# Monash-Connected-Autonomous-Vehicle/unsupervised-pseuso-LiDAR

Hardware: AMD Instinct MI355X
Metric: images/sec (fwd+bwd) KITTI 192x640 triplets, full training step (higher is better)
Workload: dtype f32; 1 GPU; BASELINE.json configs[1]: per-GPU batch=12, 192x640 KITTI-shaped triplets, ResNet-18 depth encoder + 6-DoF PoseNet, fp32 (the ResNet trunk's 3x3 stride-1 convolutions and their data gradients: fp32 contractions on split operands -- three bf16 planes per operand, six bf16-MFMA plane products, fp32 accumulation; every other launch: fp32 MFMA), one step = 2x depth fwd + pose fwd + warp/L1/smooth loss; global_batch=12, parallelism=dp1

## Files before the change

### unsupervised-pseuso-lidar_amd/csrc/conv_bf16.hip

```cpp
#include "conv_shared.h"
#include "kernel_timer.h"

namespace mcav {

typedef __bf16 bf16x8 __attribute__((ext_vector_type(8)));
typedef __bf16 bf16x4 __attribute__((ext_vector_type(4)));
typedef __bf16 bf16x2 __attribute__((ext_vector_type(2)));
typedef unsigned short u16;
typedef unsigned int u32x2 __attribute__((ext_vector_type(2)));

template <int BM_, int BN_, int WM_, int WN_, int MF_, int CK_>
struct BTile {
    static constexpr int BM = BM_, BN = BN_, WM = WM_, WN = WN_, MF = MF_;
    static constexpr int KD = CK_;
    static constexpr int LDH = CK_ + 8;
    static constexpr int LPRA = CK_ / 4;
    static constexpr int RPPA = 256 / LPRA;
    static constexpr int AROWS = BM / RPPA;
    static constexpr int LPRB = CK_ / 8;
    static constexpr int BVECS = (BN * LPRB + 255) / 256;
    static constexpr int WAVES_M = BM / WM, WAVES_N = BN / WN;
    static constexpr int TM = WM / MF, TN = WN / MF;
    static constexpr int ACC = MF == 32 ? 16 : 4;
    using AccT = typename std::conditional<MF_ == 32, f32x16, f32x4>::type;
// ... 750 lines not shown
            const bf16x8 zero = {0, 0, 0, 0, 0, 0, 0, 0};
#pragma unroll
            for (int q = 0; q < NS; ++q) {
                const bf16x8 v = *reinterpret_cast<const bf16x8*>(ap + q * APL);
                a[q] = keep ? v : zero;
            }
        };
        const bool yrow = (ky == 0 && has_y1) || (ky == 2 && has_yl);
        const unsigned ybit = ky == 0 ? 1u : 2u;
        const int sky = 2 - ky;
        for (int ks = 0; ks < 2; ++ks) {
            bf16x8 b[3][NS];
#pragma unroll
            for (int kx = 0; kx < 3; ++kx)
#pragma unroll
                for (int q = 0; q < NS; ++q) b[kx][q] = *reinterpret_cast<const bf16x8*>(Bst + (ks ? b_lane1 : b_lane0) + (kx * NS + q) * BPL);
            const unsigned m = rmask;
            bf16x8 a[NS];
            if (has_x1) { afr(ky, 2, ks, a, (m & 4u) != 0); mma(a, b[0]); }
            if (has_xl) { afr(ky, 0, ks, a, (m & 8u) != 0); mma(a, b[2]); }
            if (yrow) {
                const bool my = (m & ybit) != 0;
#pragma unroll
                for (int kx = 0; kx < 3; ++kx) { afr(sky, kx, ks, a, my); mma(a, b[kx]); }
                if (has_x1) { afr(sky, 2, ks, a, my && (m & 4u)); mma(a, b[0]); }
                if (has_xl) { afr(sky, 0, ks, a, my && (m & 8u)); mma(a, b[2]); }
            }
        }
    };
    auto compute = [&](int ky, const u16* Bst) {
        const int rsh = (fwd ? ky : 2 - ky) * PW + (fwd ? 0 : 2);
        const int dxr = fwd ? 1 : -1;
        bf16x8 fa[2][NS], fb[2][NS];
        auto load = [&](int i, bf16x8 (&a)[NS], bf16x8 (&b)[NS]) {
            const int kx = i >> 1, ks = i & 1;
            const u16* const bp = Bst + (ks ? b_lane1 : b_lane0) + kx * NS * BPL;
#pragma unroll
            for (int q = 0; q < NS; ++q) b[q] = *reinterpret_cast<const bf16x8*>(bp + q * BPL);
            const int row = prow + rsh + kx * dxr;
            const u16* const ap = Asub + row * LDH + (((2 * ks + fslot) ^ ((row >> 2) & 3)) * 8);
#pragma unroll
            for (int q = 0; q < NS; ++q) a[q] = *reinterpret_cast<const bf16x8*>(ap + q * APL);
        };
        load(0, fa[0], fb[0]);
#pragma unroll
        for (int i = 0; i < 6; ++i) {
            if (i + 1 < 6) load(i + 1, fa[(i + 1) & 1], fb[(i + 1) & 1]);
            __builtin_amdgcn_sched_barrier(0);
            if (!(diag & 8)) mma(fa[i & 1], fb[i & 1]);
            __builtin_amdgcn_sched_barrier(0);
        }
    };

    f32x4 ra[NJ], rbn[NS];
    const int total = nchunks * 3;
    issueA(ra, 0);
    issueB(rbn, 0);
    storeA(ra);
    storeB(rbn, 0);
    if (total > 1) issueB(rbn, 1);
    __syncthreads();
    int ky = 0, chunk = 0;
    for (int s = 0; s < total; ++s) {
        const bool more = chunk + 1 < nchunks;
        const u16* const Bst = Bs + (s & 1) * BSTAGE;
        if (ky == 0 && more && !(diag & 4)) issueA(ra, chunk + 1);
        compute(ky, Bst);
        if constexpr (ADJ) {
            if (has_y1 | has_yl | has_x1 | has_xl) extras(ky, Bst);
        }
        if (s + 1 < total && !(diag & 1)) {
            storeB(rbn, (s + 1) & 1);
            if (s + 2 < total) issueB(rbn, s + 2);
        }
        if (ky == 2 && more && !(diag & 4)) {
            __syncthreads();
            storeA(ra);
        }
        __syncthreads();
        if (++ky == 3) { ky = 0; ++chunk; }
    }
    if constexpr (NS > 1) acc[0][0] += mid + low;
    if (diag & 16) return;
    igemm_epilogue_lean<T>(p, acc, s_out, s_stat, tid, wm0, wn0, n0, mt);
}

#ifndef MCAV_PATCH2_DIAG
#define MCAV_PATCH2_DIAG 0
#endif

template <int SB, int BN_>
struct Patch2Cfg {
    static constexpr int BM = 64 * SB, BN = BN_;
    static constexpr int PIX = 110;
    static constexpr int VP = SB * PIX;
    static constexpr int NJ = (VP + 31) / 32;
    using T = typename std::conditional<SB == 4, BTile<256, BN_, 64, BN_, 32, 32>, BTile<128, BN_, 32, BN_, 32, 32>>::type;
};

template <int NS, int SB, int BN>
constexpr size_t patch2_lds_bytes() { return sizeof(u16) * (size_t)NS * (SB * 110 + 2 * 3 * BN) * 32 + sizeof(unsigned) * 64 * SB; }

template <int NS, int SB, int BN>
__global__ __launch_bounds__(256, BN == 32 ? 2 : 1) void conv3x3_patch2_kernel(IgemmParams p, const u16* __restrict__ w16, PatchGeo geo) {
    using C = Patch2Cfg<SB, BN>;
    using T = typename C::T;
    constexpr int BM = C::BM, CKT = 32, LDH = 32, PIX = C::PIX, TM = T::TM, TN = T::TN;
    constexpr int APL = PIX * LDH;
    constexpr int BPL = BN * LDH;
    constexpr int BSTAGE = 3 * NS * BPL;
    extern __shared__ __attribute__((aligned(16))) unsigned char s_raw[];
    u16* const Ap = reinterpret_cast<u16*>(s_raw);
    u16* const Bs = Ap + SB * NS * APL;
    unsigned* const s_out = reinterpret_cast<unsigned*>(Bs + 2 * BSTAGE);
    float (*const s_stat)[2][BN] = reinterpret_cast<float (*)[2][BN]>(Bs);
    static_assert(sizeof(u16) * BSTAGE >= sizeof(float) * T::WAVES_M * 2 * BN, "statistics scratch fits a filter stage");

    const int tid = threadIdx.x, lane = tid & 63, wave = tid >> 6;
    const int lid = xcd_remap(blockIdx.x, gridDim.x);
    const int nt = lid % p.ntiles, mt = lid / p.ntiles;
    const int n0 = nt * BN;
    const GatherSrc& g = p.g;
    const int TH = geo.TH, TW = geo.TW, PW = TW + 2, PH = TH + 2;
    const int per_img = geo.tiles_y * geo.tiles_x, nblk = g.B * per_img;

    __shared__ int s_pp[C::PIX];
    if (tid < PIX) {
        const int ppy = tid / PW;
        s_pp[tid] = tid < PH * PW ? (ppy << 8) | (tid - ppy * PW) : -1;
    }
    int sb_base[SB], sb_y0[SB], sb_x0[SB];
#pragma unroll
    for (int sb = 0; sb < SB; ++sb) {
        const int blk = mt * SB + sb;
        const int img = blk / per_img, tr = blk - img * per_img, tyi = tr / geo.tiles_x;
        sb_base[sb] = blk < nblk ? img : -1;
        sb_y0[sb] = tyi * TH;
        sb_x0[sb] = (tr - tyi * geo.tiles_x) * TW;
    }
    {
        const int sbw = tid >> 6;
        if (sbw < SB) {
            unsigned o = OOB;
            int img = -1, y0 = 0, x0 = 0;
#pragma unroll
            for (int sb = 0; sb < SB; ++sb)
                if (sb == sbw) { img = sb_base[sb]; y0 = sb_y0[sb]; x0 = sb_x0[sb]; }
            if (img >= 0) {
                const int pix = patch_pixel(tid & 63);
                const int py = pix / TW, px = pix - py * TW;
                const int y = y0 + py, x = x0 + px;
                if (py < TH && y < p.Hd && x < p.Wd) o = (unsigned)((img * p.Hd + y) * p.Wd + x) * (unsigned)(p.Cd * 4);
            }
            s_out[tid] = o;
        }
    }
    __syncthreads();
    const int c4 = tid & 7, pp0 = tid >> 3;
    unsigned aoff[C::NJ];
#pragma unroll
    for (int j = 0; j < C::NJ; ++j) {
        const int vp = pp0 + 32 * j;
        const int sbj = vp / PIX, pp = vp - sbj * PIX;
        unsigned off = OOB;
        if (vp < C::VP) {
            int img = -1, y0 = 0, x0 = 0;
#pragma unroll
// ... 935 lines not shown
```

### unsupervised-pseuso-lidar_amd/csrc/conv_plan.h

```cpp
#pragma once
#include <stddef.h>
#include <stdlib.h>

#include "../../include/mcav_conv.h"

#ifndef MCAV_OK
#define MCAV_OK 0
#define MCAV_E_INVALID (-1)
#endif
#ifndef MCAV_KNOB_INT
#ifdef MCAV_TUNE_ENV
#define MCAV_KNOB_INT(name, dflt) ([] { const char* e = getenv(name); return e ? atoi(e) : (dflt); }())
#else
#define MCAV_KNOB_INT(name, dflt) (dflt)
#endif
#endif

namespace mcav {

constexpr int CK = 16;
constexpr int KP = 32;
constexpr int KPB = 64;
constexpr int TAB_TAPS = 32;
constexpr int WG_TABCAP = 2048;
constexpr int HT_H = 8, HT_W = 32;
constexpr int ST_TW = 32;
constexpr int ST_TH_DEPTH = 8, ST_TH_POSE = 4;
constexpr int SW_TH = 4;
constexpr int patch_pix(int tmb) { return tmb == 1 ? 110 : 180; }
constexpr int P3_SUBS = 3, P3_PIX = 110;
constexpr int WGP_PIX = 110;
static_assert(P3_PIX == patch_pix(1) && WGP_PIX == patch_pix(1), "the 64-pixel block shape of patch_plan serves every 64-pixel form");

inline int round_up(int v, int a) { return (v + a - 1) / a * a; }
inline int kstride_of(int taps, int Kp) { return round_up(taps * Kp, CK); }

constexpr void tile_dims(int id, int& BM, int& BN) {
    switch (id) {
        case 1: BM = 128; BN = 64; break;
        case 2: BM = 64; BN = 64; break;
        case 3: BM = 256; BN = 32; break;
        case 4: BM = 256; BN = 16; break;
        case 5: BM = 128; BN = 128; break;
        case 7: BM = 128; BN = 32; break;
        case 8: BM = 128; BN = 64; break;
        case 9: BM = 128; BN = 128; break;
        case 10: BM = 64; BN = 64; break;
        case 11: BM = 64; BN = 64; break;
        case 12: BM = 32; BN = 64; break;
        default: BM = 64; BN = 16; break;
    }
}
constexpr int tile_bm(int id) { int BM = 0, BN = 0; tile_dims(id, BM, BN); return BM; }
constexpr int tile_bn(int id) { int BM = 0, BN = 0; tile_dims(id, BM, BN); return BN; }
constexpr int tile_kd(int id) { return (id >= 8 && id <= 10) || id == 12 ? 32 : (id == 11 ? 64 : 16); }
constexpr int tile_arows(int id) { return tile_bm(id) * tile_kd(id) / 1024; }

struct GatherSrc {
    const float* x1;
    const float* x2;
    int B, Hs, Ws, C1, C2, up1;
    int mode, stride, sign, offset, pad_mode;
};

struct IgemmParams {
    GatherSrc g;
    const float* w;
    int kh, kw, Kp, Kstride, taps;
    float* y;
    int Hd, Wd, Cd, n_begin, n_count, y_choff;
    const float* bias;
    int act;
    const float* dact_aux;
    int dact;
    const float* addend;
    int pool;
    float* stats;
    const float *stats_x, *stats_mean, *stats_invstd;
    int M;
    int Mc, McP;
    int groups;
    int mtiles, ntiles;
    int no_tab;
    const float* wm;
    int Np_all;
    int bm;
    int upm;
    int ksplit;
    float* kslab;
};

struct PatchGeo {
    int TH, TW, tiles_y, tiles_x;
    int tmb;
    int refl;
};

struct WgradParams {
    GatherSrc g;
    int kh, kw, Kp, taps, Ktot;
    const float* dy;
    int Hd, Wd, Cdy, dy_choff, Cout;
    int CoutLoad;
    int Mpix;
    int splits, pix_per_split;
    int mtiles, ntiles;
    float* slab;
    int slabN;
    int want_bias;
    int tab_cht_log2;
    int upm;
    int Hf, Wf;
    int split_planes;
    int patch, pTH, pTW, ptiles_y, ptiles_x, prefl, pnblocks, pbps, pct_co, pnarrow;
};

struct WgradPlan {
    WgradParams p;
    int tile;
    bool use_tab;
    bool use_halo;
    bool use_stem;
    size_t slab_bytes, pre_bytes;
    int ci_t, groups, per_group;
};

struct PlanEnv {
    int cus;
};

struct IgemmRoute {
    int family;
    int variant;
    int tile;
    int mtiles, ntiles;
    int workgroups;
    int ksplit;
    PatchGeo geo;
    const mcav_igemm_desc* d;
    mcav_igemm_desc planar_d;
    IgemmParams p;
};

struct WgradRoute {
    int family;
    int variant;
    const mcav_wgrad_desc* d;
    mcav_wgrad_desc planar_d;
    WgradPlan pl;
    int workgroups;
    size_t workspace_bytes() const { return pl.slab_bytes + pl.pre_bytes; }
};

inline int pick_tile(const mcav_igemm_desc* d, long M) {
    if (d->tile) return d->tile;
    if (d->n_count <= 16) return (M >= 256 * 64 && d->kh * d->kw <= 16) ? 4 : 6;
    if (d->n_count <= 32) return 7;
    if (d->mode == MCAV_G_ADJ_REFLECT && ((M + 127) / 128) * ((d->n_count + 63) / 64) >= 1024) return 2;
    if (d->mode != MCAV_G_SMALLC && ((M + 127) / 128) * ((d->n_count + 63) / 64) >= 1024) return 1;
    const long t64 = ((M + 63) / 64) * ((d->n_count + 63) / 64);
    if (d->mode != MCAV_G_SMALLC && d->Kp % 32 == 0 && (t64 <= 128 || (t64 > 256 && t64 < 512))) return 12;
    if (d->mode != MCAV_G_SMALLC && d->Kp % 32 == 0) return 10;
    const long t128x64 = ((M + 127) / 128) * ((d->n_count + 63) / 64);
    return t128x64 >= 1024 ? 1 : 2;
}

inline bool bytes_fit_31(long a, long b, long c, long e) {
    const long lim = 0x7fffffffL;
    if (a <= 0 || b <= 0 || c <= 0 || e <= 0) return false;
    if (a >= lim / b) return false;
    a *= b;
    if (a >= lim / c) return false;
    a *= c;
    return a < lim / e;
}

inline bool prod_below(long lim, long a, long b, long c = 1, long e = 1) { return (unsigned __int128)a * b * c * e < (unsigned __int128)lim; }

inline bool fill_params(const mcav_igemm_desc* d, IgemmParams& p, int& tile) {
    if (!d || !d->x1 || !d->w || !d->y) return false;
    if (d->B <= 0 || d->Hs <= 0 || d->Ws <= 0 || d->Hd <= 0 || d->Wd <= 0 || d->C1 <= 0 || d->C2 < 0) return false;
    if (d->C2 > 0 && !d->x2) return false;
    if (d->kh <= 0 || d->kw <= 0 || d->Np <= 0 || d->Kp <= 0 || d->kh > 64 || d->kw > 64 || d->kh * d->kw > 64) return false;
    if (d->n_begin < 0 || d->n_count <= 0 || d->n_begin > d->Np - d->n_count) return false;
    if (d->Cd <= 0 || d->y_choff < 0 || d->y_choff > d->Cd - d->n_count) return false;
    if (d->mode == MCAV_G_SMALLC) { if (d->Kp != 4 || d->C1 != 4 || d->C2 != 0) return false; }
    else if (d->Kp % CK != 0 || (long)d->Kp < (long)d->C1 + d->C2) return false;
    if (d->C2 > 0 && (d->C1 % 4 != 0)) return false;
    if (d->mode == MCAV_G_ADJ_REFLECT && (d->kh != 3 || d->kw != 3 || d->Hs != d->Hd || d->Ws != d->Wd || d->Hs < 2 || d->Ws < 2)) return false;
    if (d->pad_mode == MCAV_PAD_REFLECT && (d->Hs < 2 || d->Ws < 2)) return false;
    if (d->up1 && ((d->Hs & 1) || (d->Ws & 1))) return false;
    if (d->pool && ((d->Hd & 1) || (d->Wd & 1) || d->mode == MCAV_G_ADJ_STRIDE2)) return false;
    if (d->pool && d->stats) return false;
    if (d->stats_x && (!d->stats || !d->stats_mean || !d->stats_invstd || d->pool || d->y_choff != 0 || d->n_begin != 0 || d->n_count != d->Cd)) return false;
    if (!prod_below(0x7fffffffL, d->B, d->Hs, d->Ws, (long)(d->C1 > d->C2 ? d->C1 : d->C2) * 4)) return false;
    const long kstride = ((long)d->kh * d->kw * d->Kp + CK - 1) / CK * CK;
    if (!prod_below(0x7fffffffL, d->Np, kstride, 4)) return false;
    if (!bytes_fit_31((long)d->B, d->pool ? d->Hd >> 1 : d->Hd, d->pool ? d->Wd >> 1 : d->Wd, (long)d->Cd * 4)) return false;
    p.g.x1 = d->x1; p.g.x2 = d->x2; p.g.B = d->B; p.g.Hs = d->Hs; p.g.Ws = d->Ws; p.g.C1 = d->C1; p.g.C2 = d->C2; p.g.up1 = d->up1;
    p.g.mode = d->mode; p.g.stride = d->stride; p.g.sign = d->sign; p.g.offset = d->offset; p.g.pad_mode = d->pad_mode;
    p.w = d->w; p.kh = d->kh; p.kw = d->kw; p.Kp = d->Kp; p.taps = d->kh * d->kw; p.Kstride = kstride_of(p.taps, d->Kp);
    p.y = d->y; p.Hd = d->Hd; p.Wd = d->Wd; p.Cd = d->Cd; p.n_begin = d->n_begin; p.n_count = d->n_count; p.y_choff = d->y_choff;
    p.bias = d->bias; p.act = d->act; p.dact_aux = d->dact_aux; p.dact = d->dact; p.addend = d->addend; p.pool = d->pool; p.stats = d->stats;
    p.stats_x = d->stats ? d->stats_x : nullptr; p.stats_mean = d->stats_mean; p.stats_invstd = d->stats_invstd;
    const long Mlin = (long)d->B * d->Hd * d->Wd;
    p.no_tab = (d->tile >> 8) & 1;
    p.ksplit = 1; p.kslab = nullptr;
    p.wm = d->w_upmerge; p.Np_all = d->Np; p.upm = 0; p.bm = 0;
    tile = pick_tile(d, Mlin) & 0xff;
    if (tile == 0) { mcav_igemm_desc dd = *d; dd.tile = 0; tile = pick_tile(&dd, Mlin); }
    if (((tile >= 8 && tile <= 10) || tile == 12) && (d->mode == MCAV_G_SMALLC || d->Kp % 32 != 0)) return false;
    if (tile == 11 && (d->mode == MCAV_G_SMALLC || d->Kp % 64 != 0)) return false;
    int BM, BN;
    tile_dims(tile, BM, BN);
    p.groups = d->groups > 1 ? d->groups : 1;
    if (p.groups > 1) {
        if ((d->mode != MCAV_G_DIRECT && d->mode != MCAV_G_SMALLC) || d->pool || d->B % p.groups != 0) return false;
        p.Mc = (int)(Mlin / p.groups);
        p.McP = round_up(p.Mc, BM);
        p.M = p.groups * p.McP;
    } else if (d->mode == MCAV_G_ADJ_STRIDE2) {
        p.Mc = d->B * ((d->Hd + 1) / 2) * ((d->Wd + 1) / 2);
        p.McP = round_up(p.Mc, BM);
        p.M = 4 * p.McP;
    } else {
        p.Mc = 0; p.McP = 1;
        if (Mlin > 0x7fffffffL) return false;
        p.M = (int)Mlin;
        const int ck = tile_kd(tile);
        if (d->w_upmerge && d->mode == MCAV_G_DIRECT && d->kh == 3 && d->kw == 3 && d->stride == 1 && d->sign == 1 && d->offset == -1 &&
            d->pad_mode == MCAV_PAD_REFLECT && d->up1 == 1 && d->C2 > 0 && !(d->Hd & 1) && !(d->Wd & 1) && d->Hd == d->Hs && d->Wd == d->Ws &&
            !d->pool && !d->stats && d->C1 % ck == 0 && d->C2 % ck == 0 && d->C1 + d->C2 == d->Kp && (d->C1 & 3) == 0 && !p.no_tab &&
            (long)4 * d->Np * 4 * d->C1 * 4 < 0x7fffffffL) {
            p.upm = 1;
            p.bm = BM;
            p.Mc = d->B * (d->Hd / 2) * (d->Wd / 2);
            p.McP = round_up(p.Mc, BM);
            p.M = 4 * p.McP;
        }
    }
    p.mtiles = (p.M + BM - 1) / BM;
    p.ntiles = (d->n_count + BN - 1) / BN;
    return true;
}

inline void plan_fp32(IgemmRoute& r) {
    const IgemmParams& p = r.p;
    const int KD = tile_kd(r.tile), AROWS = tile_arows(r.tile);
    const bool c4ok = (p.g.C1 & 3) == 0 && (p.g.C2 & 3) == 0 && (p.g.C2 == 0 || (p.g.C1 & 15) == 0);
    const bool fast_mode = p.g.mode == MCAV_G_DIRECT || (p.g.mode == MCAV_G_ADJ_STRIDE2 && p.g.C2 == 0) || p.g.mode == MCAV_G_SMALLC;
    const bool tab = (p.g.mode == MCAV_G_DIRECT || (p.g.mode == MCAV_G_ADJ_STRIDE2 && p.g.C2 == 0)) && c4ok && p.taps <= TAB_TAPS &&
                     p.g.C1 + p.g.C2 == p.Kp && p.Kp % KD == 0 && (p.g.C2 == 0 || p.g.C1 % KD == 0) && !p.no_tab;
    const bool tab_refl = p.g.mode == MCAV_G_ADJ_REFLECT && c4ok && p.g.C2 == 0 && p.g.C1 == p.Kp && p.Kp % KD == 0 && !p.no_tab && AROWS <= 2;
    r.family = MCAV_IGEMM_FP32;
    r.ksplit = 1;
    if (p.upm) r.variant = MCAV_RV_TABLE | MCAV_RV_UPM;
    else if (tab) r.variant = MCAV_RV_TABLE;
    else if (tab_refl) r.variant = MCAV_RV_TABLE | MCAV_RV_REFLECT | MCAV_RV_ADJ;
    else if (fast_mode && c4ok) r.variant = MCAV_RV_FAST;
    else if (p.g.mode == MCAV_G_ADJ_REFLECT && c4ok && p.g.C2 == 0) r.variant = MCAV_RV_REFLECT | MCAV_RV_ADJ;
    else r.variant = 0;
    if (tab && !p.upm) {
        const bool plain = !p.pool && !p.stats && p.groups <= 1 && p.y_choff == 0 && p.n_count == p.Cd && p.n_begin == 0;
        const int tiles = p.mtiles * p.ntiles, ktiles = p.Kp / KD * p.taps;
        static const int enabled = MCAV_KNOB_INT("MCAV_KSPLIT", 1);
        static const int max_tiles = MCAV_KNOB_INT("MCAV_KSPLIT_TILES", 256);
        if (enabled && plain && tiles <= max_tiles && ktiles >= 32) {
            int ksp = 1024 / tiles;
            if (ksp > 8) ksp = 8;
            if (ksp > ktiles / 4) ksp = ktiles / 4;
            if (ksp >= 2) r.ksplit = ksp;
        }
    }
    r.mtiles = p.mtiles; r.ntiles = p.ntiles;
    r.workgroups = p.mtiles * p.ntiles * r.ksplit;
}

inline bool plan_halo(const mcav_igemm_desc* d, IgemmRoute& r) {
    if (d->kh != 3 || d->kw != 3 || d->stride != 1) return false;
    if (d->C2 != 0 || d->x2 || (d->C1 != 16 && d->C1 != 32) || d->Kp != d->C1) return false;
    if (d->n_count > 32 || d->stats || d->groups > 1 || d->y_choff != 0) return false;
    if (d->Hd != d->Hs || d->Wd != d->Ws || d->Hs < 2 || d->Ws < 2) return false;
    if ((d->tile >> 9) & 1) return false;
    const bool adj = d->mode == MCAV_G_ADJ_REFLECT;
    if (adj) {
        if (d->dact & ~0xff) return false;
        if (d->up1 || d->bias || d->act != MCAV_ACT_NONE) return false;
        if (d->pool && ((d->Hs & 1) || (d->Ws & 1))) return false;
    } else {
        if (d->mode != MCAV_G_DIRECT || d->sign != 1 || d->offset != -1) return false;
// ... 39 lines not shown
        for (int i = 0; i < ns; ++i)
            if (!d->x_planar[i]) return -1;
        return 1;
    }
    if (kind == 2) return d->planar_stack == 2 && d->planar_B == d->B && d->x_planar[1] && d->x_planar[2] ? 1 : -1;
    return -1;
}

inline bool plan_stem(const mcav_igemm_desc* d, bool planar, IgemmRoute& r) {
    const int kind = stem_kind(d);
    if (!kind) return false;
    const int th = kind == 1 ? ST_TH_DEPTH : ST_TH_POSE;
    r.family = MCAV_IGEMM_STEM;
    r.mtiles = d->B * ((d->Hd + th - 1) / th) * ((d->Wd + ST_TW - 1) / ST_TW);
    r.ntiles = 1;
    static const int split_on = MCAV_KNOB_INT("MCAV_STEM_SPLIT", 0);
    const bool split = kind == 1 && (d->mma == 3 || (d->mma == 2 && split_on));
    const bool lean = ((d->tile >> 16) & 1) || kind == 2;
    r.variant = (kind == 2 ? MCAV_RV_POSE : 0) | (planar ? MCAV_RV_PLANAR : 0) | (split ? MCAV_RV_SPLIT : 0) | (lean ? MCAV_RV_LEAN : 0);
    r.workgroups = r.mtiles < (split ? 256 : 512) ? r.mtiles : (split ? 256 : 512);
    return true;
}

inline double patch_block(int H, int W, int rows, int pix, int& TH, int& TW) {
    double best = 1e30;
    TH = 4; TW = 16;
    for (int th = 1; th <= 16; ++th)
        for (int tw = 4; tw <= 64; ++tw) {
            if (th * tw > rows || (th + 2) * (tw + 2) > pix) continue;
            const double tiles = (double)((H + th - 1) / th) * ((W + tw - 1) / tw);
            const double bank = tw % 16 == 0 ? 1.0 : (tw > 16 && tw % 4 == 0 ? 1.05 : 1.25);
            const double cost = tiles * rows * (1.0 + 0.05 * (double)((th + 2) * (tw + 2)) / (th * tw)) * bank;
            if (cost < best) { best = cost; TH = th; TW = tw; }
        }
    return best;
}

struct PatchPlan {
    PatchGeo geo;
    int th1, tw1;
};

inline bool patch_plan(const mcav_igemm_desc* d, PatchPlan& pp, bool f32 = false) {
    PatchGeo& geo = pp.geo;
    static const int enabled = MCAV_KNOB_INT("MCAV_PATCH", 1);
    if (!enabled || !d) return false;
    if (f32 ? (d->mma != 0 || !d->w) : (!d->w16 || d->mma < 1 || d->mma > 3)) return false;
    if (d->kh != 3 || d->kw != 3 || d->stride != 1) return false;
    geo.refl = 0;
    if (d->mode == MCAV_G_DIRECT && d->pad_mode == MCAV_PAD_REFLECT && d->sign == 1 && d->offset == -1) geo.refl = 1;
    else if (d->mode == MCAV_G_ADJ_REFLECT && d->sign == -1 && d->offset == 1) geo.refl = 2;
    else if (d->mode != MCAV_G_DIRECT || d->pad_mode != MCAV_PAD_ZERO) return false;
    else if (!((d->sign == 1 && d->offset == -1) || (d->sign == -1 && d->offset == 1))) return false;
    static const int refl_on = MCAV_KNOB_INT("MCAV_PATCH_REFLECT", 1);
    if (geo.refl && (f32 || d->mma < 2 || !refl_on || d->Hs < 2 || d->Ws < 2)) return false;
    static const int refl_minpix = MCAV_KNOB_INT("MCAV_PATCH_REFLECT_MINPIX", 1000);
    if (geo.refl && d->mma != 3 && (d->n_count < 64 || (geo.refl == 2 && d->Hd * d->Wd < refl_minpix))) return false;
    if (d->C2 != 0 || d->up1 || d->pool || d->w_upmerge) return false;
    if (d->C1 % 32 != 0 || d->Kp != d->C1 || d->Hd != d->Hs || d->Wd != d->Ws || d->n_count < 32) return false;
    if (d->groups > 1 && d->B % d->groups != 0) return false;
    static const int force_tmb = MCAV_KNOB_INT("MCAV_PATCH_TMB", 0);
    int th2, tw2;
    const double c1 = patch_block(d->Hd, d->Wd, 64, patch_pix(1), pp.th1, pp.tw1);
    const double c2 = patch_block(d->Hd, d->Wd, 128, patch_pix(2), th2, tw2);
    const long wg2 = (long)d->B * ((d->Hd + th2 - 1) / th2) * ((d->Wd + tw2 - 1) / tw2) * ((d->n_count + 63) / 64);
    geo.tmb = (c2 <= c1 * 1.02 && wg2 >= 1024) ? 2 : 1;
    if (force_tmb == 1 || force_tmb == 2) geo.tmb = force_tmb;
    geo.TH = geo.tmb == 2 ? th2 : pp.th1;
    geo.TW = geo.tmb == 2 ? tw2 : pp.tw1;
    geo.tiles_y = (d->Hd + geo.TH - 1) / geo.TH;
    geo.tiles_x = (d->Wd + geo.TW - 1) / geo.TW;
    if (d->mma == 1 && (long)d->B * geo.tiles_y * geo.tiles_x * ((d->n_count + 63) / 64) < 1024) return false;
    return true;
}

inline PatchGeo patch_geo64(const mcav_igemm_desc* d, const PatchPlan& pp) {
    PatchGeo geo = pp.geo;
    geo.TH = pp.th1; geo.TW = pp.tw1; geo.tmb = 1;
    geo.tiles_y = (d->Hd + geo.TH - 1) / geo.TH;
    geo.tiles_x = (d->Wd + geo.TW - 1) / geo.TW;
    return geo;
}

inline bool patch3_plan(const mcav_igemm_desc* d, bool patch, const PatchPlan& pp, PatchGeo& geo) {
    static const int enabled = MCAV_KNOB_INT("MCAV_PATCH3", 0);
    static const int min_wgs = MCAV_KNOB_INT("MCAV_PATCH3_MIN_WGS", 192);
    static const int min_k = MCAV_KNOB_INT("MCAV_PATCH3_MIN_K", 128);
    if (d->mma < 2) return false;
    const bool forced = (d->tile & 0xff) == 0x33;
    if ((!enabled && !forced) || !patch) return false;
    geo = patch_geo64(d, pp);
    const long nblk = (long)d->B * geo.tiles_y * geo.tiles_x;
    if (d->groups > 1 && (nblk / d->groups) % P3_SUBS != 0) return false;
    const long wgs = ((nblk + P3_SUBS - 1) / P3_SUBS) * ((d->n_count + 63) / 64);
    if (!forced && (wgs < min_wgs || d->Kp < min_k)) return false;
    return true;
}

inline int patch2_plan(const mcav_igemm_desc* d, bool patch, const PatchPlan& pp, const PlanEnv& env, PatchGeo& geo, int& bn) {
    static const int enabled = MCAV_KNOB_INT("MCAV_PATCH2", 0);
    static const int force_sb = MCAV_KNOB_INT("MCAV_PATCH2_SB", 0);
    static const int force_bn = MCAV_KNOB_INT("MCAV_PATCH2_BN", 0);
    if (d->mma < 2) return 0;
    if (!enabled && !((d->tile >> 14) & 3)) return 0;
    if (!patch || pp.geo.refl) return 0;
    geo = patch_geo64(d, pp);
    const long per_img = (long)geo.tiles_y * geo.tiles_x, nblk = d->B * per_img, ntiles = (d->n_count + 63) / 64;
    const int groups = (d->stats && d->groups > 1) ? d->groups : 1;
    const int cus = env.cus;
    auto fits = [&](int sb) { return d->B % groups == 0 && ((d->B / groups) * per_img) % sb == 0; };
    auto cost = [&](int sb) { const long wgs = ((nblk + sb - 1) / sb) * ntiles; return ((wgs + cus - 1) / cus) * sb; };
    int sb = 0;
    if (fits(4)) sb = 4;
    if (fits(2) && (sb == 0 || cost(2) < cost(4))) sb = 2;
    if ((force_sb == 2 || force_sb == 4) && fits(force_sb)) sb = force_sb;
    bn = 64;
    if ((force_bn == 32 || ((d->tile >> 15) & 1)) && fits(2)) { sb = 2; bn = 32; }
    return sb;
}

inline int bf16_tile_for(const mcav_igemm_desc* d, bool patch, bool* refl) {
    if (!d || !d->w16 || (d->mma < 1 || d->mma > 3)) return 0;
    if (d->mma == 2 && !patch) return 0;
    if (d->pool || d->w_upmerge) return 0;
    if ((long)d->kh * d->kw > TAB_TAPS || d->Kp % 32 != 0 || (long)d->C1 + d->C2 != d->Kp) return 0;
    if ((d->C1 & 3) || (d->C2 & 3) || (d->C2 > 0 && d->C1 % 32 != 0)) return 0;
    if (d->n_count < 32) return 0;
    if (d->C2 == 0 && d->C1 <= 32 && d->n_count <= 32 && d->kh == 3 && d->stride == 1) return 0;
    const bool direct = d->mode == MCAV_G_DIRECT || (d->mode == MCAV_G_ADJ_STRIDE2 && d->C2 == 0);
    const bool radj = d->mode == MCAV_G_ADJ_REFLECT && d->C2 == 0;
    if (!direct && !radj) return 0;
    *refl = radj;
    const bool k64 = d->mma == 1 && d->Kp % 64 == 0 && (d->C2 == 0 || d->C1 % 64 == 0);
    const long M = (long)d->B * d->Hd * d->Wd;
    const long wg64 = ((M + 63) / 64) * ((d->n_count + 63) / 64);
    int shape = 10;
    if (wg64 >= 4096 && !radj) shape = 8;
    else if (wg64 < 512) shape = 12;
    if (d->mma >= 2) {
        static const int forced = MCAV_KNOB_INT("MCAV_SPLIT_TILE", 0);
        if ((forced == 10 || forced == 12 || (forced == 8 && !radj))) shape = forced;
    }
    return shape * 2 + (k64 ? 1 : 0);
}

inline bool igemm_uses_bf16(const mcav_igemm_desc* d) {
    PatchPlan pp;
    bool refl = false;
    return bf16_tile_for(d, d && d->mma == 2 && patch_plan(d, pp), &refl) != 0;
}

inline bool patch_rows(const mcav_igemm_desc* d, int tile_id, long blocks, int bn, IgemmRoute& r) {
    mcav_igemm_desc dd = *d;
    dd.tile = tile_id;
    if (!fill_params(&dd, r.p, r.tile)) return false;
    r.p.mtiles = r.mtiles = (int)blocks;
    r.p.ntiles = r.ntiles = (r.p.n_count + bn - 1) / bn;
    r.workgroups = r.mtiles * r.ntiles;
    return true;
}

inline bool plan_patch_f32(const mcav_igemm_desc* d, IgemmRoute& r) {
    static const int enabled = MCAV_KNOB_INT("MCAV_PATCH_F32", 0);
    if (!enabled && !((d->tile >> 13) & 1)) return false;
    PatchPlan pp;
    if (!patch_plan(d, pp, true)) return false;
    r.geo = pp.geo;
    if (!patch_rows(d, 2, (long)d->B * r.geo.tiles_y * r.geo.tiles_x, 64, r)) return false;
    r.family = MCAV_IGEMM_PATCH_F32;
    r.variant = r.geo.tmb == 2 ? MCAV_RV_TMB2 : 0;
    return true;
}

inline int plan_bf16(const mcav_igemm_desc* d, const PlanEnv& env, IgemmRoute& r) {
    PatchPlan pp;
    const bool patch = patch_plan(d, pp);
    bool refl = false;
    const int bt = bf16_tile_for(d, patch, &refl);
    if (!bt) return 1;
    const bool split = d->mma >= 2;
    int bn2 = 64;
    bool ok;
    if (patch3_plan(d, patch, pp, r.geo)) {
        const long nblk = (long)d->B * r.geo.tiles_y * r.geo.tiles_x;
        ok = patch_rows(d, 10, (nblk + P3_SUBS - 1) / P3_SUBS, 64, r);
        r.family = MCAV_IGEMM_BF16_PATCH3;
        r.variant = MCAV_RV_SPLIT | (r.geo.refl == 2 ? MCAV_RV_ADJ | MCAV_RV_REFLECT : r.geo.refl == 1 ? MCAV_RV_REFLECT : 0);
    } else if (const int sb = patch2_plan(d, patch, pp, env, r.geo, bn2)) {
        const long nblk = (long)d->B * r.geo.tiles_y * r.geo.tiles_x;
        ok = patch_rows(d, 10, (nblk + sb - 1) / sb, bn2, r);
        r.family = MCAV_IGEMM_BF16_PATCH2;
        r.variant = MCAV_RV_SPLIT | (sb == 4 ? MCAV_RV_SB4 : 0) | (bn2 == 32 ? MCAV_RV_BN32 : 0);
    } else if (patch) {
        r.geo = pp.geo;
        ok = patch_rows(d, 10, (long)d->B * r.geo.tiles_y * r.geo.tiles_x, 64, r);
        r.family = MCAV_IGEMM_BF16_PATCH;
        r.variant = (split ? MCAV_RV_SPLIT : 0) | (r.geo.tmb == 2 ? MCAV_RV_TMB2 : 0) | (r.geo.refl == 2 ? MCAV_RV_ADJ | MCAV_RV_REFLECT : r.geo.refl == 1 ? MCAV_RV_REFLECT : 0);
    } else {
        mcav_igemm_desc dd = *d;
        dd.tile = bt >> 1;
        ok = fill_params(&dd, r.p, r.tile) && (r.tile == 8 || r.tile == 10 || r.tile == 12);
        r.family = MCAV_IGEMM_BF16_TILE;
        r.variant = (split ? MCAV_RV_SPLIT : 0) | ((bt & 1) ? MCAV_RV_K64 : 0) | (refl ? MCAV_RV_ADJ | MCAV_RV_REFLECT : 0);
        r.mtiles = r.p.mtiles; r.ntiles = r.p.ntiles;
        r.workgroups = r.mtiles * r.ntiles;
    }
    if (!ok) return MCAV_E_INVALID;
    if ((long)d->Np * r.p.Kstride * 2 * (split ? 3 : 1) >= 0x7fffffffL) return MCAV_E_INVALID;
    return MCAV_OK;
}

inline int plan_igemm(const mcav_igemm_desc* d, const PlanEnv& env, IgemmRoute& r, bool halo = true) {
    r.family = MCAV_IGEMM_FP32; r.variant = r.tile = r.mtiles = r.ntiles = r.workgroups = 0; r.ksplit = 1; r.geo = PatchGeo{};
    const int planar = stem_planar_state(d, stem_kind(d));
    if (planar < 0) return MCAV_E_INVALID;
    if (planar && !d->x1) { r.planar_d = *d; r.planar_d.x1 = d->x_planar[0]; d = &r.planar_d; }
    r.d = d;
    if (!fill_params(d, r.p, r.tile)) return MCAV_E_INVALID;
    r.mtiles = r.p.mtiles; r.ntiles = r.p.ntiles;
    if (planar) return plan_stem(d, true, r) ? MCAV_OK : MCAV_E_INVALID;
    if (halo && plan_halo(d, r)) {
        IgemmRoute next;
        r.mtiles = plan_igemm(d, env, next, false) == MCAV_OK ? next.mtiles : r.p.mtiles;
        return MCAV_OK;
    }
    if (plan_stem(d, false, r)) return MCAV_OK;
    if (plan_patch_f32(d, r)) return MCAV_OK;
    if (d->mma != 0) {
        const int rc = plan_bf16(d, env, r);
        if (rc != 1) return rc;
    }
    plan_fp32(r);
    return MCAV_OK;
}

inline int halo_wgrad_splits(const mcav_wgrad_desc* d) {
    if (d->mode != MCAV_G_DIRECT || d->kh != 3 || d->kw != 3 || d->stride != 1 || d->sign != 1 || d->offset != -1) return 0;
    if (d->C2 != 0 || d->x2 || (d->C1 != 16 && d->C1 != 32) || d->Kp != d->C1 || d->Cin != d->C1) return 0;
    if (d->Cout > 32 || (d->C1 == 32 && d->Cout > 16)) return 0;
    if (d->Hd != d->Hs || d->Wd != d->Ws || d->Hs < 2 || d->Ws < 2) return 0;
    if ((d->Cdy & 3) || (d->dy_choff & 3) || ((d->tile >> 9) & 1)) return 0;
    const int cl = (d->Cout + 3) / 4 * 4;
    if (cl > d->Cdy - d->dy_choff) return 0;
    const long tiles = (long)d->B * ((d->Hs + HT_H - 1) / HT_H) * ((d->Ws + HT_W - 1) / HT_W);
    return (int)(tiles < 512 ? tiles : 512);
}

inline int stem_wgrad_splits(const mcav_wgrad_desc* d) {
    if (!stem_wgrad_kind(d)) return 0;
    const long tiles = (long)d->B * ((d->Hd + SW_TH - 1) / SW_TH) * ((d->Wd + ST_TW - 1) / ST_TW);
    return (int)(tiles < 512 ? tiles : 512);
}

inline int stem_wgrad_bn(const mcav_wgrad_desc* d) {
    if (!d) return 0;
    if (!d->dy_bn_x && !d->dy_bn_gamma && !d->dy_bn_mean && !d->dy_bn_invstd && !d->dy_bn_sums && !d->dy_bn_groups && d->dy_bn_inv_count == 0.f) return 0;
    if (stem_wgrad_kind(d) != 1 || d->dbias) return -1;
    if (d->dy_choff != 0 || d->Cdy != 64) return -1;
    if (!d->dy_bn_x || !d->dy_bn_gamma || !d->dy_bn_mean || !d->dy_bn_invstd || !d->dy_bn_sums) return -1;
    if (d->dy_bn_groups < 1 || d->B % d->dy_bn_groups || !(d->dy_bn_inv_count > 0.f)) return -1;
    return 1;
}

inline int wgrad_fill_splits(int Mpix, int out_tiles, int slots, int max_splits, int ktile) {
    auto wgs_of = [&](int sp) {
        const int pps = round_up((Mpix + sp - 1) / sp, ktile);
        return out_tiles * ((Mpix + pps - 1) / pps);
    };
// ... 240 lines not shown
```

### unsupervised-pseuso-lidar_amd/csrc/conv_shared.h

```cpp
#pragma once
#include <stdlib.h>
#include <type_traits>
#include <utility>

#include "conv_gather.h"

namespace mcav {

template <int BM_, int BN_, int WM_, int WN_, int MF_, int CK_ = 16>
struct Tile {
    static constexpr int BM = BM_, BN = BN_, WM = WM_, WN = WN_, MF = MF_;
    static constexpr int KD = CK_;
    static constexpr int LD = CK_ + 4;
    static constexpr int LPR = CK_ / 4;
    static constexpr int RPP = 256 / LPR;
    static constexpr int WAVES_M = BM / WM, WAVES_N = BN / WN;
    static constexpr int TM = WM / MF, TN = WN / MF;
    static constexpr int ACC = MF == 32 ? 16 : 4;
    using AccT = typename std::conditional<MF_ == 32, f32x16, f32x4>::type;
    static constexpr int AROWS = BM / RPP;
    static constexpr int BVECS = (BN * LPR + 255) / 256;
    static_assert(WAVES_M * WAVES_N == 4, "4 wavefronts per workgroup");
    static_assert(BM % RPP == 0, "BM multiple of the rows per pass");
};
// ... 74 lines not shown
    constexpr int BN = T::BN;
    const int lane = tid & 63, wave = tid >> 6;
    constexpr int MF = T::MF;
    const int ccol = lane & (MF - 1);
    float ssum[T::TN], ssq[T::TN];
#pragma unroll
    for (int j = 0; j < T::TN; ++j) { ssum[j] = 0.f; ssq[j] = 0.f; }
#pragma unroll
    for (int i = 0; i < T::TM; ++i)
#pragma unroll
        for (int j = 0; j < T::TN; ++j) {
            const int nl = n0 + wn0 + j * MF + ccol;
            const bool ncol = nl < p.n_count;
            const float bv = (p.bias && ncol) ? p.bias[p.n_begin + nl] : 0.f;
#pragma unroll
            for (int q = 0; q < T::ACC / 4; ++q) {
                const int rbase = wm0 + i * MF + (MF == 32 ? 8 * q + 4 * (lane >> 5) : 4 * (lane >> 4));
                float v[4];
#pragma unroll
                for (int e = 0; e < 4; ++e) v[e] = act_fwd(acc[i][j][4 * q + e] + bv, p.act);
                if (p.pool) {
                    const int o = s_out[rbase];
                    if (o >= 0 && ncol) {
                        float s = (v[0] + v[1]) + (v[2] + v[3]);
                        const size_t off = (size_t)o * p.Cd + p.y_choff + nl;
                        if (p.dact_aux && !(p.dact & MCAV_DACT_AFTER_ADDEND)) s *= act_bwd(p.dact_aux[off], p.dact & 0xff);
                        if (p.addend) s += p.addend[off];
                        if (p.dact_aux && (p.dact & MCAV_DACT_AFTER_ADDEND)) s *= act_bwd(p.dact_aux[off], p.dact & 0xff);
                        p.y[off] = s;
                    }
                } else {
#pragma unroll
                    for (int e = 0; e < 4; ++e) {
                        const int o = s_out[rbase + e];
                        if (o >= 0 && ncol) {
                            float s = v[e];
                            const size_t off = (size_t)o * p.Cd + p.y_choff + nl;
                            if (p.dact_aux && !(p.dact & MCAV_DACT_AFTER_ADDEND)) s *= act_bwd(p.dact_aux[off], p.dact & 0xff);
                            if (p.addend) s += p.addend[off];
                            if (p.dact_aux && (p.dact & MCAV_DACT_AFTER_ADDEND)) s *= act_bwd(p.dact_aux[off], p.dact & 0xff);
                            p.y[off] = s;
                            ssum[j] += s;
                            if (p.stats_x) {
                                const int gi = (mt / (p.mtiles / p.groups)) * p.n_count + nl;
                                ssq[j] += s * ((p.stats_x[off] - p.stats_mean[gi]) * p.stats_invstd[gi]);
                            } else {
                                ssq[j] += s * s;
                            }
                        }
                    }
                }
            }
        }
    if (p.stats) {
#pragma unroll
        for (int j = 0; j < T::TN; ++j) {
            if (MF == 32) {
                ssum[j] += __shfl_xor(ssum[j], 32, 64);
                ssq[j] += __shfl_xor(ssq[j], 32, 64);
            } else {
                ssum[j] += __shfl_xor(ssum[j], 16, 64); ssq[j] += __shfl_xor(ssq[j], 16, 64);
                ssum[j] += __shfl_xor(ssum[j], 32, 64); ssq[j] += __shfl_xor(ssq[j], 32, 64);
            }
            if (lane < MF) {
                s_stat[wave / T::WAVES_N][0][wn0 + j * MF + lane] = ssum[j];
                s_stat[wave / T::WAVES_N][1][wn0 + j * MF + lane] = ssq[j];
            }
        }
        __syncthreads();
        for (int e = tid; e < 2 * BN; e += 256) {
            const int which = e / BN, col = e - which * BN;
            if (n0 + col < p.n_count) {
                float s = 0.f;
#pragma unroll
                for (int wmi = 0; wmi < T::WAVES_M; ++wmi) s += s_stat[wmi][which][col];
                p.stats[((size_t)mt * 2 + which) * p.n_count + n0 + col] = s;
            }
        }
    }
}

template <class T>
__device__ __forceinline__ void igemm_epilogue_lean(const IgemmParams& p, typename T::AccT (&acc)[T::TM][T::TN], const unsigned* s_outb,
                                                    float (*s_stat)[2][T::BN], int tid, int wm0, int wn0, int n0, int mt) {
    constexpr int BN = T::BN, MF = T::MF, NQ = T::ACC / 4;
    const int lane = tid & 63, wave = tid >> 6;
    const int ccol = lane & (MF - 1);
    const unsigned ybytes = (unsigned)((size_t)p.g.B * (p.pool ? (p.Hd >> 1) * (p.Wd >> 1) : p.Hd * p.Wd) * p.Cd * 4);
    const __amdgpu_buffer_rsrc_t ry = make_rsrc(p.y, ybytes);
    const __amdgpu_buffer_rsrc_t rx = make_rsrc(p.dact_aux ? p.dact_aux : p.y, ybytes);
    const __amdgpu_buffer_rsrc_t rad = make_rsrc(p.addend ? p.addend : p.y, ybytes);
    const __amdgpu_buffer_rsrc_t rsx = make_rsrc(p.stats_x ? p.stats_x : p.y, ybytes);
    const int sgrp = p.stats_x ? (mt / (p.mtiles / p.groups)) * p.n_count : 0;
    float ssum[T::TN], ssq[T::TN];
#pragma unroll
    for (int j = 0; j < T::TN; ++j) { ssum[j] = 0.f; ssq[j] = 0.f; }
#pragma unroll
    for (int i = 0; i < T::TM; ++i)
#pragma unroll
        for (int j = 0; j < T::TN; ++j) {
            __builtin_amdgcn_sched_barrier(0);
            const int nl = n0 + wn0 + j * MF + ccol;
            if (nl < p.n_count) {
                const float bv = p.bias ? p.bias[p.n_begin + nl] : 0.f;
                const unsigned colb = (unsigned)(p.y_choff + nl) * 4u;
                u32x4 ro[NQ];
#pragma unroll
                for (int q = 0; q < NQ; ++q) {
                    const int rbase = wm0 + i * MF + (MF == 32 ? 8 * q + 4 * (lane >> 5) : 4 * (lane >> 4));
                    ro[q] = *reinterpret_cast<const u32x4*>(&s_outb[rbase]);
                }
                if (p.pool) {
                    float aux[NQ], add[NQ];
                    if (p.dact_aux) {
#pragma unroll
                        for (int q = 0; q < NQ; ++q) aux[q] = buf_load1(rx, ro[q].x + colb);
                    }
                    if (p.addend) {
#pragma unroll
                        for (int q = 0; q < NQ; ++q) add[q] = buf_load1(rad, ro[q].x + colb);
                    }
#pragma unroll
                    for (int q = 0; q < NQ; ++q) {
                        float v[4];
#pragma unroll
                        for (int e = 0; e < 4; ++e) v[e] = act_fwd(acc[i][j][4 * q + e] + bv, p.act);
                        float s = (v[0] + v[1]) + (v[2] + v[3]);
                        if (p.dact_aux && !(p.dact & MCAV_DACT_AFTER_ADDEND)) s *= act_bwd(aux[q], p.dact & 0xff);
                        if (p.addend) s += add[q];
                        if (p.dact_aux && (p.dact & MCAV_DACT_AFTER_ADDEND)) s *= act_bwd(aux[q], p.dact & 0xff);
                        buf_store1(ry, ro[q].x + colb, s);
                    }
                } else {
                    constexpr int QH = NQ >= 2 ? NQ / 2 : 1;
#pragma unroll
                    for (int q0 = 0; q0 < NQ; q0 += QH) {
                        float aux[4 * QH], add[4 * QH], xs[4 * QH];
                        float smu = 0.f, sis = 0.f;
                        if (p.stats_x) {
                            smu = p.stats_mean[sgrp + nl];
                            sis = p.stats_invstd[sgrp + nl];
#pragma unroll
                            for (int q = 0; q < QH; ++q)
#pragma unroll
                                for (int e = 0; e < 4; ++e) xs[4 * q + e] = buf_load1(rsx, ro[q0 + q][e] + colb);
                        }
                        if (p.dact_aux) {
#pragma unroll
                            for (int q = 0; q < QH; ++q)
#pragma unroll
                                for (int e = 0; e < 4; ++e) aux[4 * q + e] = buf_load1(rx, ro[q0 + q][e] + colb);
                        }
                        if (p.addend) {
#pragma unroll
                            for (int q = 0; q < QH; ++q)
#pragma unroll
                                for (int e = 0; e < 4; ++e) add[4 * q + e] = buf_load1(rad, ro[q0 + q][e] + colb);
                        }
#pragma unroll
                        for (int q = 0; q < QH; ++q)
#pragma unroll
                            for (int e = 0; e < 4; ++e) {
                                float s = acc[i][j][4 * (q0 + q) + e] + bv;
                                if (p.act == MCAV_ACT_RELU) s = fmaxf(s, 0.f);
                                else if (p.act != MCAV_ACT_NONE) s = act_fwd(s, p.act);
                                if (p.dact_aux && !(p.dact & MCAV_DACT_AFTER_ADDEND)) s *= act_bwd(aux[4 * q + e], p.dact & 0xff);
                                if (p.addend) s += add[4 * q + e];
                                if (p.dact_aux && (p.dact & MCAV_DACT_AFTER_ADDEND)) s *= act_bwd(aux[4 * q + e], p.dact & 0xff);
                                buf_store1(ry, ro[q0 + q][e] + colb, s);
                                if (p.stats) {
                                    const float sv = ro[q0 + q][e] != OOB ? s : 0.f;
                                    ssum[j] += sv;
                                    ssq[j] += p.stats_x ? sv * ((xs[4 * q + e] - smu) * sis) : sv * sv;
                                }
                            }
                        __builtin_amdgcn_sched_barrier(0);
                    }
                }
            }
        }
    if (p.stats) {
#pragma unroll
        for (int j = 0; j < T::TN; ++j) {
            if (MF == 32) {
                ssum[j] += __shfl_xor(ssum[j], 32, 64);
                ssq[j] += __shfl_xor(ssq[j], 32, 64);
            } else {
                ssum[j] += __shfl_xor(ssum[j], 16, 64); ssq[j] += __shfl_xor(ssq[j], 16, 64);
                ssum[j] += __shfl_xor(ssum[j], 32, 64); ssq[j] += __shfl_xor(ssq[j], 32, 64);
            }
            if (lane < MF) {
                s_stat[wave / T::WAVES_N][0][wn0 + j * MF + lane] = ssum[j];
                s_stat[wave / T::WAVES_N][1][wn0 + j * MF + lane] = ssq[j];
            }
        }
        __syncthreads();
        for (int e = tid; e < 2 * BN; e += 256) {
            const int which = e / BN, col = e - which * BN;
            if (n0 + col < p.n_count) {
                float s = 0.f;
#pragma unroll
                for (int wmi = 0; wmi < T::WAVES_M; ++wmi) s += s_stat[wmi][which][col];
                p.stats[((size_t)mt * 2 + which) * p.n_count + n0 + col] = s;
            }
        }
    }
}

}
```

Before: 1156 images/s.

## Enable patch3 bf16 conv kernel by default for forward split-precision convolutions

Result: no change. 1158 images/s, median of 6 (+0.1%).

```diff
diff --git a/unsupervised-pseuso-lidar_amd/csrc/conv_bf16.hip b/unsupervised-pseuso-lidar_amd/csrc/conv_bf16.hip
--- a/unsupervised-pseuso-lidar_amd/csrc/conv_bf16.hip
+++ b/unsupervised-pseuso-lidar_amd/csrc/conv_bf16.hip
@@ -856,7 +856,8 @@
     }
     if constexpr (NS > 1) acc[0][0] += mid + low;
     if (diag & 16) return;
-    igemm_epilogue_lean<T>(p, acc, s_out, s_stat, tid, wm0, wn0, n0, mt);
+    static_assert(T::WAVES_M * T::WAVES_N * 64 == P3_THREADS && T::WAVES_M % P3_SUBS == 0, "a statistics row per block: two wavefront rows each");
+    igemm_epilogue_lean<T>(p, acc, s_out, s_stat, tid, wm0, wn0, n0, mt, p.stat_rows, nblocks);
 }
 
 #ifndef MCAV_PATCH2_DIAG
diff --git a/unsupervised-pseuso-lidar_amd/csrc/conv_plan.h b/unsupervised-pseuso-lidar_amd/csrc/conv_plan.h
--- a/unsupervised-pseuso-lidar_amd/csrc/conv_plan.h
+++ b/unsupervised-pseuso-lidar_amd/csrc/conv_plan.h
@@ -88,6 +88,7 @@
     int upm;
     int ksplit;
     float* kslab;
+    int stat_rows;
 };
 
 struct PatchGeo {
@@ -205,7 +206,7 @@
     p.stats_x = d->stats ? d->stats_x : nullptr; p.stats_mean = d->stats_mean; p.stats_invstd = d->stats_invstd;
     const long Mlin = (long)d->B * d->Hd * d->Wd;
     p.no_tab = (d->tile >> 8) & 1;
-    p.ksplit = 1; p.kslab = nullptr;
+    p.ksplit = 1; p.kslab = nullptr; p.stat_rows = 1;
     p.wm = d->w_upmerge; p.Np_all = d->Np; p.upm = 0; p.bm = 0;
     tile = pick_tile(d, Mlin) & 0xff;
     if (tile == 0) { mcav_igemm_desc dd = *d; dd.tile = 0; tile = pick_tile(&dd, Mlin); }
@@ -411,19 +412,23 @@
     return geo;
 }
 
-inline bool patch3_plan(const mcav_igemm_desc* d, bool patch, const PatchPlan& pp, PatchGeo& geo) {
+enum { P3_OPT_IN = 1, P3_FORWARD = 2 };
+inline int patch3_plan(const mcav_igemm_desc* d, bool patch, const PatchPlan& pp, PatchGeo& geo) {
     static const int enabled = MCAV_KNOB_INT("MCAV_PATCH3", 0);
+    static const int fwd_on = MCAV_KNOB_INT("MCAV_PATCH3_FWD", 1);
     static const int min_wgs = MCAV_KNOB_INT("MCAV_PATCH3_MIN_WGS", 192);
     static const int min_k = MCAV_KNOB_INT("MCAV_PATCH3_MIN_K", 128);
-    if (d->mma < 2) return false;
+    if (d->mma < 2 || !patch) return 0;
     const bool forced = (d->tile & 0xff) == 0x33;
-    if ((!enabled && !forced) || !patch) return false;
+    const bool pinned = (d->tile & 0xff) != 0 || ((d->tile >> 14) & 3);
+    const bool forward = fwd_on && d->mma == 2 && d->sign > 0 && !pinned && pp.geo.tmb == 1 && pp.geo.refl == 0;
+    if (!enabled && !forced && !forward) return 0;
     geo = patch_geo64(d, pp);
     const long nblk = (long)d->B * geo.tiles_y * geo.tiles_x;
-    if (d->groups > 1 && (nblk / d->groups) % P3_SUBS != 0) return false;
+    if (d->groups > 1 && (nblk / d->groups) % P3_SUBS != 0) return 0;
     const long wgs = ((nblk + P3_SUBS - 1) / P3_SUBS) * ((d->n_count + 63) / 64);
-    if (!forced && (wgs < min_wgs || d->Kp < min_k)) return false;
-    return true;
+    if (!forced && (wgs < min_wgs || d->Kp < min_k)) return 0;
+    return (enabled || forced) ? P3_OPT_IN : P3_FORWARD;
 }
 
 inline int patch2_plan(const mcav_igemm_desc* d, bool patch, const PatchPlan& pp, const PlanEnv& env, PatchGeo& geo, int& bn) {
@@ -510,9 +515,13 @@
     const bool split = d->mma >= 2;
     int bn2 = 64;
     bool ok;
-    if (patch3_plan(d, patch, pp, r.geo)) {
+    if (const int p3 = patch3_plan(d, patch, pp, r.geo)) {
         const long nblk = (long)d->B * r.geo.tiles_y * r.geo.tiles_x;
         ok = patch_rows(d, 10, (nblk + P3_SUBS - 1) / P3_SUBS, 64, r);
+        if (p3 == P3_FORWARD) {
+            r.p.stat_rows = P3_SUBS;
+            r.mtiles = (int)nblk;
+        }
         r.family = MCAV_IGEMM_BF16_PATCH3;
         r.variant = MCAV_RV_SPLIT | (r.geo.refl == 2 ? MCAV_RV_ADJ | MCAV_RV_REFLECT : r.geo.refl == 1 ? MCAV_RV_REFLECT : 0);
     } else if (const int sb = patch2_plan(d, patch, pp, env, r.geo, bn2)) {
diff --git a/unsupervised-pseuso-lidar_amd/csrc/conv_shared.h b/unsupervised-pseuso-lidar_amd/csrc/conv_shared.h
--- a/unsupervised-pseuso-lidar_amd/csrc/conv_shared.h
+++ b/unsupervised-pseuso-lidar_amd/csrc/conv_shared.h
@@ -180,7 +180,8 @@
 
 template <class T>
 __device__ __forceinline__ void igemm_epilogue_lean(const IgemmParams& p, typename T::AccT (&acc)[T::TM][T::TN], const unsigned* s_outb,
-                                                    float (*s_stat)[2][T::BN], int tid, int wm0, int wn0, int n0, int mt) {
+                                                    float (*s_stat)[2][T::BN], int tid, int wm0, int wn0, int n0, int mt, int srows = 1,
+                                                    int srow_end = 0) {
     constexpr int BN = T::BN, MF = T::MF, NQ = T::ACC / 4;
     const int lane = tid & 63, wave = tid >> 6;
     const int ccol = lane & (MF - 1);
@@ -293,6 +294,19 @@
             }
         }
         __syncthreads();
+        if (srows > 1) {
+            const int wpr = T::WAVES_M / srows;
+            for (int e = tid; e < 2 * BN * srows; e += T::WAVES_M * T::WAVES_N * 64) {
+                const int r = e / (2 * BN), which = (e / BN) & 1, col = e % BN;
+                const int row = mt * srows + r;
+                if (n0 + col < p.n_count && row < srow_end) {
+                    float s = 0.f;
+                    for (int k = 0; k < wpr; ++k) s += s_stat[r * wpr + k][which][col];
+                    p.stats[((size_t)row * 2 + which) * p.n_count + n0 + col] = s;
+                }
+            }
+            return;
+        }
         for (int e = tid; e < 2 * BN; e += 256) {
             const int which = e / BN, col = e - which * BN;
             if (n0 + col < p.n_count) {
```
